# WGLab/DeepMod

Hardware: AMD Instinct MI355X
Metric: base-positions/sec (whole node), E. coli 5mC wd21/f7 BiLSTM (higher is better)
Workload: dtype f16x3

## Files before the change

### deepmod_amd/_lib.py

```python
from __future__ import annotations

import ctypes
import os
from typing import Optional

os.environ.setdefault("HSA_ENABLE_IPC_MODE_LEGACY", "0")

HERE = os.path.dirname(os.path.abspath(__file__))
LIB_PATH = os.path.join(HERE, "csrc", "libdeepmod_hip.so")

DM_OPT_PROFILE = 1
DM_OPT_PRECISION = 2
DM_OPT_ASYNC = 3
DM_OPT_RESERVED_CUS = 4
DM_OPT_F16X3_SHAPE = 5
DM_PREC_F32 = 0
DM_PREC_F16X3 = 1
DM_PREC_F16I8 = 3
DM_PREC_F16X3_ROLES = 2
DM_INFO_PRECISION, DM_INFO_F16_REPRESENTABLE, DM_INFO_F16_LENGTH_SHIFT, DM_INFO_DEVICE, DM_INFO_HAS_F16X3_ROLES = 1, 2, 3, 4, 5
DM_INFO_HAS_F16S = 6
DM_OK, DM_EINVAL, DM_EDEVICE, DM_ENOMEM, DM_ESTATE, DM_ERCCL, DM_ERANGE = 0, -1, -2, -3, -4, -5, -6
(DM_MAP_STATUS, DM_MAP_N_ROWS, DM_MAP_LEFTCLIP, DM_MAP_RIGHTCLIP, DM_MAP_EV_LO, DM_MAP_EV_HI, DM_MAP_FIRST_MATCH_POS,
 DM_MAP_LAST_MATCH_POS, DM_MAP_NUM_INSERT, DM_MAP_NUM_DELETE, DM_MAP_NUM_MISMATCH, DM_MAP_STRAND, DM_MAP_POS_AFTER_CLIP,
 DM_MAP_EVENTS_AFTER_CLIP) = range(14)
DM_MAP_INFO_LEN = 16
DM_MAP_OK, DM_MAP_NO_MATCH, DM_MAP_NEED_ROWS = 0, 1, 2
DM_MOVE_OK, DM_MOVE_COUNT, DM_MOVE_OUTSIDE = 0, 1, 2
(DM_XY_OK, DM_XY_LESS_EVENT, DM_XY_NO_SITE, DM_XY_FILTERED, DM_XY_NO_MATCH, DM_XY_INDEX_ERROR, DM_XY_NEED_ROWS) = range(7)
DM_XY_INFO_LEN = 8
(DM_XY_STATUS, DM_XY_N_ROWS, DM_XY_STRAND, DM_XY_START_CLIP, DM_XY_END_CLIP, DM_XY_POS_AFTER_CLIP, DM_XY_EVENTS_AFTER_CLIP) = range(7)
DM_WEIGHT_FLOATS = 408402

_c = ctypes
_vp = ctypes.c_void_p
_i64 = ctypes.c_int64
# ... 167 lines not shown
```

### deepmod_amd/csrc/deepmod_hip.hip

```cpp
#include "kernels.h"

#include <dlfcn.h>
#include <rccl/rccl.h>

#include <algorithm>
#include <cmath>
#include <cstdarg>
#include <cstdint>
#include <cstdio>
#include <cstring>
#include <string>
#include <utility>
#include <thread>
#include <type_traits>
#include <vector>

#include "../../include/deepmod_hip.h"
#include "head.hip.inc"

using dmk::Packed16;
using dmk::Packed32;

namespace {

// ... 886 lines not shown
}

int dm_model_sync(dm_model* m) {
    if (!m) return fail(DM_EINVAL, "null model");
    HIP_TRY(hipSetDevice(m->device));
    return sync_and_check(m);
}

int dm_model_get_info(dm_model* m, int key, int64_t* value) {
    if (!m || !value) return fail(DM_EINVAL, "null argument");
    switch (key) {
        case DM_INFO_PRECISION: *value = m->precision; return DM_OK;
        case DM_INFO_F16_REPRESENTABLE: *value = m->f16_ok ? 1 : 0; return DM_OK;
        case DM_INFO_F16_LENGTH_SHIFT: *value = m->len_shift; return DM_OK;
        case DM_INFO_DEVICE: *value = m->device; return DM_OK;
        case DM_INFO_HAS_F16S:
#ifdef DM_WITH_F16S
            *value = 1;
#else
            *value = 0;
#endif
            return DM_OK;
        case DM_INFO_HAS_F16X3_ROLES:
#ifdef DM_WITH_F16X3_ROLES
            *value = 1;
#else
            *value = 0;
#endif
            return DM_OK;
        default: return fail(DM_EINVAL, "unknown info key %d", key);
// ... 630 lines not shown
```

### deepmod_amd/csrc/kernels.h

```cpp
#pragma once
#include <hip/hip_runtime.h>

#if defined(DM16Q_ABL_NOCELL) || defined(DM16Q_ABL_NODMA) || defined(DM16Q_ABL_MIX1) || defined(DM16Q_ABL_I8T) || defined(DM16Q_ABL_NOBAR) || defined(DM16Q_ABL_NOVMWAIT) || defined(DM16Q_AINIT) || defined(DM16Q_DEBUG_NOP) ||           \
    defined(DM16Q_NOCHUNK) || defined(DM16Q_NOPN) || defined(DM16Q_LOPACK) || defined(DM16Q_PRE) || defined(DM16Q_SNAKE) || defined(DM16Q_TRANS_COST) ||                     \
    defined(DM16S_ABL_2PROD) || defined(DM16S_ABL_B64) || defined(DM16S_ABL_LO_ONLY) || defined(DM16S_ABL_MFMA16) ||                              \
    defined(DM16S_ABL_MFMA16_PAD) || defined(DM16S_ABL_NOBAR) || defined(DM16S_ABL_NOCELL) || defined(DM16S_ABL_NODMA) ||                          \
    defined(DM16S_ABL_NOLDSA) || defined(DM16S_ADIST) || defined(DM16S_ALO_TRUNC) || defined(DM16S_PRE) || defined(DM_ABL_NOBAR) ||                \
    defined(DM_ABL_NODMA) || defined(DM_ABL_NOEPI) || defined(DM_ABL_NOSEQ) || defined(DM_TIMING) || defined(DM_TRACE) || defined(DM_TRACE2) ||   \
    defined(DM_WLO_TRUNC_ENV) || defined(DM_WLO_TRUNC_DEFAULT) || defined(DM_WITH_F16X3_ROLES) || defined(DM16R_DMA_M) ||                         \
    defined(DM_F16X3_SHAPE_DEFAULT) || defined(DM_WAVES) || defined(DM_MT) || defined(DM_WITH_F16S)
#define DM_ANY_EXPERIMENT_SWITCH 1
#ifndef DM_EXPERIMENT
#error "an ablation / experiment macro is defined without -DDM_EXPERIMENT: timing-only kernels must not be built into the product by a stray -D"
#endif
#else
#define DM_ANY_EXPERIMENT_SWITCH 0
#endif


#if defined(DM_WITH_F16X3_ROLES) && !defined(DM_WITH_F16S)
#error "the roles experiment lives in the translation unit of the 32x32x16 kernels: build it with -DDM_WITH_F16S as well"
#endif

#include <algorithm>
// ... 94 lines not shown
```

### deepmod_amd/csrc/lstm_f16q.hip.inc

```
#ifndef DM16Q_TRANS_COST
#define DM16Q_TRANS_COST 2
#endif
namespace lstm16q {

using lstmc::floatx2;
using lstmc::floatx4;
using lstmc::halfx2;
using lstmc::halfx8;
using lstmc::uintx4;
using lstmc::Params;
using lstmc::ex2;
using lstmc::rcp;
using lstmc::min60;
using lstmc::split_pack;
using lstmc::static_for;
using lstmc::as_h8;

constexpr int HID = 100, NFEAT = 7, WIN = 21, LIVE = 11;
constexpr int NTILE = 13;
constexpr int WAVES = 4, THREADS = 64 * WAVES, TILE_M = 32 * WAVES;
constexpr int KS_L0 = 4, KS_L12 = 7;
constexpr int REC_BYTES = 4096;
constexpr int MIX_BYTES = 2048;
constexpr int TILE_BYTES_L0 = (KS_L0 - 1) * REC_BYTES + 2 * MIX_BYTES, TILE_BYTES_L12 = (KS_L12 - 1) * REC_BYTES + MIX_BYTES;
constexpr int SLOT_BYTES = TILE_BYTES_L12;
constexpr int NSLOT = 2;
constexpr int C2_WAVE_BYTES = NTILE * 1024;
constexpr int C2_LAYER_BYTES = WAVES * C2_WAVE_BYTES;
constexpr size_t LDS_BYTES = size_t(NSLOT) * SLOT_BYTES + C2_LAYER_BYTES;
constexpr size_t LDS_BYTES_I8 = LDS_BYTES + C2_LAYER_BYTES;
constexpr size_t WEIGHT_BYTES_DIR = size_t(NTILE) * (TILE_BYTES_L0 + 2 * TILE_BYTES_L12);
constexpr size_t WEIGHT_BYTES = 2 * WEIGHT_BYTES_DIR;

using lstmc::intx4;
using lstmc::I8_MAGIC;
using lstmc::I8_HI_SCALE;
using lstmc::I8_LO_SCALE;
struct CellPipe {
    float ef[4], ei[4], ej[4], eo[4], t0[4], t1[4];
    unsigned hi01, hi23, lo01, lo23, i01, i23;
    floatx2 fold[2];
    floatx2 kmagic, khi, klo;
    static constexpr int NM = 14;
    template <int PRE, int FMT>
    __device__ static constexpr int nops(int M) {
// ... 142 lines not shown
        return;
#endif
        if constexpr (C < NCH) {
            constexpr int LO = chunk_lo<PRE, FMT>(C, NCH), HI = chunk_lo<PRE, FMT>(C + 1, NCH);
            static_for<HI - LO>([&](auto kc) {
                constexpr int k = LO + decltype(kc)::value;
                this->template op<op_m<PRE, FMT>(k), op_j<PRE, FMT>(k), FMT>(g, gi, S, c2, only_a);
            });
        }
    }
    template <int PRE, int FMT>
    __device__ __forceinline__ void all(floatx4 (&g)[4], const intx4 (&gi)[4], const floatx2 (&S)[2], float* c2, const bool only_a) { chunk<0, 1, PRE, FMT>(g, gi, S, c2, only_a); }
};

template <int TILE_BYTES>
__device__ __forceinline__ void stage_tile(const unsigned char* gtile , unsigned lds_slot , int wave_s, unsigned lane16) {
#ifdef DM16Q_ABL_NODMA
    return;
#endif
    constexpr int NKB = TILE_BYTES / 1024, BASE = NKB / WAVES, REM = NKB % WAVES;
    static_assert(TILE_BYTES % 1024 == 0 && BASE >= 1 && BASE + (REM ? 1 : 0) <= 7, "pieces per wave");
    const int kb0 = wave_s * BASE + (wave_s < REM ? wave_s : REM);
    const unsigned char* g = gtile + kb0 * 1024 + 4096;
    const unsigned l = lds_slot + unsigned(kb0) * 1024u + 4096u;
    unsigned keep;
    asm volatile("s_mov_b32 %0, m0\n\ts_mov_b32 m0, %1\n\ts_nop 0" : "=&s"(keep) : "s"(l) : "memory");
#define DM_PIECE(J) if constexpr ((J) < BASE) asm volatile("global_load_lds_dwordx4 %0, %1 offset:%2" :: "v"(lane16), "s"(g), "i"((J) * 1024 - 4096) : "memory");
    DM_PIECE(0) DM_PIECE(1) DM_PIECE(2) DM_PIECE(3) DM_PIECE(4) DM_PIECE(5) DM_PIECE(6)
#undef DM_PIECE
    if constexpr (REM > 0) {
        asm volatile("s_cmp_lt_i32 %3, %4\n\ts_cbranch_scc0 .Ldm16q_skip_%=\n\tglobal_load_lds_dwordx4 %0, %1 offset:%2\n.Ldm16q_skip_%=:"
                     :: "v"(lane16), "s"(g), "i"(BASE * 1024 - 4096), "s"(wave_s), "i"(REM) : "memory", "scc");
    }
    asm volatile("s_mov_b32 m0, %0" :: "s"(keep) : "memory");
}

struct AQuad {
    halfx8 hiA, loA, hiB, loB;
};
template <int OFF, bool WITH_B, int MIXED>
__device__ __forceinline__ void load_a(AQuad& a, const unsigned addr) {
    if constexpr (MIXED == 0) {
        asm volatile("ds_read_b128 %0, %1 offset:%2" : "=v"(a.hiA) : "v"(addr), "i"(OFF));
        asm volatile("ds_read_b128 %0, %1 offset:%2" : "=v"(a.loA) : "v"(addr), "i"(OFF + 1024));
        if constexpr (WITH_B) {
// ... 11 lines not shown
}
__host__ __device__ constexpr int a_reads(bool with_b, int mixed) { return (mixed == 1 ? 1 : 2) * (with_b ? 2 : 1); }
template <int N>
__device__ __forceinline__ void wait_a(AQuad& a) {
    asm volatile("s_waitcnt lgkmcnt(%4)" : "+v"(a.hiA), "+v"(a.loA), "+v"(a.hiB), "+v"(a.loB) : "i"(N));
}

#define DM16Q_STR2(X) #X
#define DM16Q_STR(X) DM16Q_STR2(X)
#if defined(DM16Q_NOPN)
#define DM16Q_AFTER_MFMA "s_nop " DM16Q_STR(DM16Q_NOPN)
#elif defined(DM16Q_DEBUG_NOP)
#define DM16Q_AFTER_MFMA "s_nop 15\n\ts_nop 15"
#else
#define DM16Q_AFTER_MFMA ""
#endif
#ifndef DM16Q_PRE
#define DM16Q_PRE 2
#endif

template <int LAYER, bool FIRST>
struct StageKind {
    static constexpr bool L0 = LAYER == 0;
    static constexpr int KS_FULL = L0 ? KS_L0 : KS_L12;
    static constexpr int KS = FIRST ? KS_FULL - 3 : KS_FULL;
    static constexpr int TILE_BYTES = L0 ? TILE_BYTES_L0 : TILE_BYTES_L12;
    static constexpr int DMA_OFF = FIRST ? 3 * REC_BYTES : 0;
    static constexpr int DMA_BYTES = TILE_BYTES - DMA_OFF;
    static constexpr int rec_off(int i) { return (FIRST ? 3 + i : i) * REC_BYTES; }
    static constexpr int mixed(int i) { return i == KS - 1 ? (L0 ? 2 : 1) : 0; }
// ... 3 lines not shown

constexpr int quad(int t, int hh, int part) { return (t * 2 + hh) * 2 + part; }

struct WaveState {
    uintx4 own[3][12];
    unsigned m12[3][2][2];
    uintx4 nxt[12];
    float c2reg[NTILE][4];
    float c1reg[NTILE][4];
    floatx4 acc[3][4];
    intx4 acci[3][4];
    floatx2 i8s[3][2];
    CellPipe cp;
    float xf[2][2];
    int slot;
};

template <int LAYER, int MM>
__device__ __forceinline__ void c2_load(WaveState& w, const unsigned c2lds, const int tile, float (&row)[4]) {
    if constexpr (LAYER == 2) {
#pragma unroll
        for (int q = 0; q < 4; ++q) row[q] = w.c2reg[tile][q];
    } else if constexpr (LAYER == 1 && MM == 0) {
#pragma unroll
        for (int q = 0; q < 4; ++q) row[q] = w.c1reg[tile][q];
    } else {
        floatx4 v;
        asm volatile("ds_read_b128 %0, %1 offset:%2" : "=v"(v) : "v"(c2lds), "i"(LAYER * C2_LAYER_BYTES));
#pragma unroll
        for (int q = 0; q < 4; ++q) row[q] = v[q];
    }
// ... 2 lines not shown
__device__ __forceinline__ void c2_store(WaveState& w, const unsigned c2lds, const int tile, const float (&row)[4]) {
    if constexpr (LAYER == 2) {
#pragma unroll
        for (int q = 0; q < 4; ++q) w.c2reg[tile][q] = row[q];
    } else if constexpr (LAYER == 1 && MM == 0) {
#pragma unroll
        for (int q = 0; q < 4; ++q) w.c1reg[tile][q] = row[q];
    } else {
        asm volatile("ds_write_b128 %0, %1 offset:%2" :: "v"(c2lds), "v"(floatx4{row[0], row[1], row[2], row[3]}), "i"(LAYER * C2_LAYER_BYTES) : "memory");
    }
}

__device__ __forceinline__ unsigned lo_lo(unsigned a, unsigned b) { return __builtin_amdgcn_perm(b, a, 0x05040100u); }
__device__ __forceinline__ unsigned hi_lo(unsigned a, unsigned b) { return __builtin_amdgcn_alignbit(b, a, 16); }

template <int LAYER, bool FIRST, int MM>
__device__ __forceinline__ void run_stage(const Params& p, WaveState& w, const unsigned lds_base, const unsigned c2_wave, const unsigned char* wdir, const int dir, const int s,
                                          const float* xwin0, const float* xwin1, const int wave_s, const unsigned lane16, const int grp, const unsigned one2) {
    using K = StageKind<LAYER, FIRST>;
    constexpr bool L0 = K::L0;
    constexpr int KS = K::KS;
    constexpr int PREV = (LAYER + 2) % 3;
    constexpr int I8 = (MM == 1 && !(L0 && FIRST)) ? 1 : 0;
    constexpr int PRE = I8;
    constexpr int PPRE = (MM == 1 && !(PREV == 0 && FIRST)) ? 1 : 0;
    constexpr int FMT = MM == 0 ? 0 : (LAYER == 2 ? 2 : 1);
    constexpr size_t LAYER_OFF[3] = {0, size_t(NTILE) * TILE_BYTES_L0, size_t(NTILE) * (TILE_BYTES_L0 + TILE_BYTES_L12)};
    uintx4 (&own)[12] = w.own[LAYER];
    const uintx4 (&inp)[12] = w.own[L0 ? 0 : LAYER - 1];
    const floatx2 (&S)[2] = w.i8s[LAYER];
    const floatx2 (&PS)[2] = w.i8s[PREV];
    uintx4 mx[2], mx2[2];
    unsigned x0p[2] = {0u, 0u}, x1a[2] = {0u, 0u}, x1b[2] = {0u, 0u};
    if constexpr (L0) {
        bool bad = false;
#pragma unroll
        for (int hh = 0; hh < 2; ++hh) {
// ... 14 lines not shown
        if (bad) *p.range_flag = 1;
        if (s + 1 < LIVE) {
            const int row = dir == 0 ? s + 1 : WIN - 2 - s;
            const int f1 = 4 + grp < NFEAT ? 4 + grp : NFEAT - 1;
            w.xf[0][0] = xwin0[row * NFEAT + grp]; w.xf[0][1] = xwin0[row * NFEAT + f1];
            w.xf[1][0] = xwin1[row * NFEAT + grp]; w.xf[1][1] = xwin1[row * NFEAT + f1];
        }
    }
    const bool last_stage = LAYER == 2 && s == LIVE - 1;
    static_for<NTILE>([&](auto Tc) {
        constexpr int T = decltype(Tc)::value;
        constexpr int P = T == 0 ? NTILE - 1 : T - 1;
        constexpr int accT = T == NTILE - 1 ? 2 : (T & 1), accP = P == NTILE - 1 ? 2 : (P & 1);
        constexpr bool WITH_B = T < NTILE - 1;
        constexpr int NMF = (WITH_B ? 4 : 2) * (I8 ? 2 : 3);
        float c2row[4];
        if constexpr (T == 0) c2_load<PREV, MM>(w, c2_wave + unsigned(NTILE - 1) * 1024u, NTILE - 1, c2row);
        else c2_load<LAYER, MM>(w, c2_wave + unsigned(P) * 1024u, P, c2row);
        const unsigned a_addr = lds_base + unsigned(w.slot) * SLOT_BYTES + lane16;
#ifdef DM16Q_AINIT
        AQuad a[2] = {};
#else
        AQuad a[2];
#endif
        load_a<K::rec_off(0), WITH_B, K::mixed(0)>(a[0], a_addr);
        if (!(last_stage && T == NTILE - 1)) {
            if constexpr (T + 1 < NTILE) {
                unsigned toff = unsigned(T + 1) * K::TILE_BYTES;
                asm volatile("" : "+s"(toff));
                stage_tile<K::DMA_BYTES>(wdir + (LAYER_OFF[LAYER] + K::DMA_OFF) + toff, lds_base + unsigned(w.slot ^ 1) * SLOT_BYTES + K::DMA_OFF, wave_s, lane16);
            } else {
                using KN = StageKind<(LAYER + 1) % 3, FIRST && LAYER < 2>;
                stage_tile<KN::DMA_BYTES>(wdir + (LAYER_OFF[(LAYER + 1) % 3] + KN::DMA_OFF), lds_base + unsigned(w.slot ^ 1) * SLOT_BYTES + KN::DMA_OFF, wave_s, lane16);
            }
        }
        floatx4 (&d)[4] = w.acc[accT];
        intx4 (&di)[4] = w.acci[accT];
        floatx4 (&g)[4] = w.acc[accP];
        const intx4 (&gi)[4] = w.acci[accP];
        const floatx4 z4 = {0.f, 0.f, 0.f, 0.f};
        const intx4 zi4 = {0, 0, 0, 0};
        constexpr int NCH = DM16Q_PRE + NMF * (KS - 1);
#ifdef DM16Q_NOCHUNK
#define DM_CHUNK(C) do { if constexpr ((C) == NCH - 1) { if constexpr (T == 0) w.cp.template all<PPRE, 0>(g, gi, PS, c2row, true); else w.cp.template all<PRE, FMT>(g, gi, S, c2row, false); } } while (0)
#else
#define DM_CHUNK(C) do { if constexpr (T == 0) w.cp.template chunk<(C), NCH, PPRE, 0>(g, gi, PS, c2row, true); else w.cp.template chunk<(C), NCH, PRE, FMT>(g, gi, S, c2row, false); } while (0)
#endif
        if constexpr (KS > 1) static_for<DM16Q_PRE>([&](auto cc) { DM_CHUNK(decltype(cc)::value); });
        static_for<KS>([&](auto ic) {
            constexpr int i = decltype(ic)::value;
            constexpr int MIXED = K::mixed(i);
            if constexpr (i + 1 < KS) load_a<K::rec_off(i + 1), WITH_B, K::mixed(i + 1)>(a[(i + 1) & 1], a_addr);
            if constexpr (i == KS - 1) {
                if constexpr (KS == 1) {
                    if constexpr (T == 0) w.cp.template all<PPRE, 0>(g, gi, PS, c2row, true);
                    else w.cp.template all<PRE, FMT>(g, gi, S, c2row, false);
                }
#ifdef DM16Q_ABL_NOCELL
                w.cp.hi01 = w.cp.hi23 = 0x2E662E66u; w.cp.lo01 = w.cp.lo23 = 0x0A660A66u;
#endif
                if constexpr (T == 0) {
                    w.m12[PREV][0][0] = lo_lo(w.cp.hi01, w.cp.hi01); w.m12[PREV][0][1] = lo_lo(w.cp.hi01, w.cp.lo01);
                    w.m12[PREV][1][0] = lo_lo(w.cp.hi23, w.cp.hi23); w.m12[PREV][1][1] = lo_lo(w.cp.hi23, w.cp.lo23);
                    c2_store<PREV, MM>(w, c2_wave + unsigned(NTILE - 1) * 1024u, NTILE - 1, c2row);
                } else {
                    constexpr int pt = P >> 2, pr = P & 3;
                    unsigned s01, s23;
// ... 14 lines not shown
                    }
                });
            }
            if constexpr (MIXED != 0 && T == 0) {
#pragma unroll
                for (int hh = 0; hh < 2; ++hh) {
                    unsigned in_hl;
                    if constexpr (L0) in_hl = x0p[hh];
                    else in_hl = w.m12[LAYER - 1][hh][1];
                    unsigned own_hh = w.m12[LAYER][hh][0], own_hl = w.m12[LAYER][hh][1];
                    asm volatile("" : "+v"(own_hh), "+v"(own_hl), "+v"(in_hl));
                    mx[hh] = uintx4{own_hh, hi_lo(own_hl, in_hl), in_hl, one2};
                    if constexpr (L0) mx2[hh] = uintx4{x1a[hh], x1b[hh], 0u, 0u};
                }
            }
            wait_a<(i + 1 < KS ? a_reads(WITH_B, K::mixed(i + 1 < KS ? i + 1 : i)) : 0)>(a[i & 1]);
            constexpr int C0 = DM16Q_PRE + NMF * i;
#define DM_MF(AOP, BOP, Q, NO)                                                                                              \
            d[Q] = __builtin_amdgcn_mfma_f32_16x16x32_f16(AOP, BOP, (i == 0 && (NO) == 0) ? z4 : d[Q], 0, 0, 0);              \
            asm volatile(DM16Q_AFTER_MFMA : "+v"(d[Q]) : "v"(AOP), "v"(BOP));
#define DM_MI(AOP, BOP, Q)                                                                                                  \
            di[Q] = __builtin_amdgcn_mfma_i32_16x16x64_i8(__builtin_bit_cast(intx4, AOP), __builtin_bit_cast(intx4, BOP), i == 0 ? zi4 : di[Q], 0, 0, 0); \
            asm volatile(DM16Q_AFTER_MFMA : "+v"(di[Q]) : "v"(AOP), "v"(BOP));
#define DM_CELLQ(N_) if constexpr (KS > 1 && i < KS - 1) DM_CHUNK(C0 + (N_))
            if constexpr (MIXED != 0) {
                const halfx8 b0 = as_h8(mx[0]), b1 = as_h8(mx[1]);
                DM_MF(a[i & 1].hiA, b0, 0, 0)
                DM_MF(a[i & 1].hiA, b1, 2, 0)
                if constexpr (WITH_B) { DM_MF(a[i & 1].hiB, b0, 1, 0) DM_MF(a[i & 1].hiB, b1, 3, 0) }
                if constexpr (MIXED == 2) {
                    const halfx8 e0 = as_h8(mx2[0]), e1 = as_h8(mx2[1]);
                    DM_MF(a[i & 1].loA, e0, 0, 1)
                    DM_MF(a[i & 1].loA, e1, 2, 1)
                    if constexpr (WITH_B) { DM_MF(a[i & 1].loB, e0, 1, 1) DM_MF(a[i & 1].loB, e1, 3, 1) }
                }
            } else {
                constexpr int t = K::opnd(i);
                halfx8 bh[2], bl[2];
#pragma unroll
                for (int hh = 0; hh < 2; ++hh) {
                    if constexpr (K::is_own(i)) { bh[hh] = as_h8(own[quad(t, hh, 0)]); bl[hh] = as_h8(own[quad(t, hh, 1)]); }
                    else { bh[hh] = as_h8(inp[quad(t, hh, 0)]); bl[hh] = as_h8(inp[quad(t, hh, 1)]); }
                }
                if constexpr (I8) {
                    DM_MF(a[i & 1].hiA, bh[0], 0, 0) DM_CELLQ(0);
                    DM_MF(a[i & 1].hiA, bh[1], 2, 0) DM_CELLQ(1);
                    if constexpr (WITH_B) { DM_MF(a[i & 1].hiB, bh[0], 1, 0) DM_CELLQ(2); DM_MF(a[i & 1].hiB, bh[1], 3, 0) DM_CELLQ(3); }
                    DM_MI(a[i & 1].loA, bl[0], 0) DM_CELLQ(WITH_B ? 4 : 2);
                    DM_MI(a[i & 1].loA, bl[1], 2) DM_CELLQ(WITH_B ? 5 : 3);
                    if constexpr (WITH_B) { DM_MI(a[i & 1].loB, bl[0], 1) DM_CELLQ(6); DM_MI(a[i & 1].loB, bl[1], 3) DM_CELLQ(7); }
                } else {
#ifdef DM16Q_SNAKE
                DM_MF(a[i & 1].hiA, bh[0], 0, 0) DM_CELLQ(0);
                if constexpr (WITH_B) { DM_MF(a[i & 1].hiB, bh[0], 1, 0) DM_CELLQ(1); DM_MF(a[i & 1].hiB, bh[1], 3, 0) DM_CELLQ(2); }
                DM_MF(a[i & 1].hiA, bh[1], 2, 0) DM_CELLQ(WITH_B ? 3 : 1);
                DM_MF(a[i & 1].loA, bh[1], 2, 1) DM_CELLQ(WITH_B ? 4 : 2);
                if constexpr (WITH_B) { DM_MF(a[i & 1].loB, bh[1], 3, 1) DM_CELLQ(5); DM_MF(a[i & 1].loB, bh[0], 1, 1) DM_CELLQ(6); }
                DM_MF(a[i & 1].loA, bh[0], 0, 1) DM_CELLQ(WITH_B ? 7 : 3);
                DM_MF(a[i & 1].hiA, bl[0], 0, 2) DM_CELLQ(WITH_B ? 8 : 4);
                if constexpr (WITH_B) { DM_MF(a[i & 1].hiB, bl[0], 1, 2) DM_CELLQ(9); DM_MF(a[i & 1].hiB, bl[1], 3, 2) DM_CELLQ(10); }
                DM_MF(a[i & 1].hiA, bl[1], 2, 2) DM_CELLQ(WITH_B ? 11 : 5);
#else
                DM_MF(a[i & 1].hiA, bh[0], 0, 0) DM_CELLQ(0);
                DM_MF(a[i & 1].hiA, bh[1], 2, 0) DM_CELLQ(1);
                if constexpr (WITH_B) { DM_MF(a[i & 1].hiB, bh[0], 1, 0) DM_CELLQ(2); DM_MF(a[i & 1].hiB, bh[1], 3, 0) DM_CELLQ(3); }
#ifdef DM16Q_ABL_I8T
                DM_MI(a[i & 1].loA, bl[0], 0) DM_CELLQ(WITH_B ? 4 : 2); DM_CELLQ(WITH_B ? 5 : 3);
                DM_MI(a[i & 1].loA, bl[1], 2) DM_CELLQ(WITH_B ? 6 : 4); DM_CELLQ(WITH_B ? 7 : 5);
                if constexpr (WITH_B) { DM_MI(a[i & 1].loB, bl[0], 1) DM_CELLQ(8); DM_CELLQ(9); DM_MI(a[i & 1].loB, bl[1], 3) DM_CELLQ(10); DM_CELLQ(11); }
#else
                DM_MF(a[i & 1].loA, bh[0], 0, 1) DM_CELLQ(WITH_B ? 4 : 2);
                DM_MF(a[i & 1].loA, bh[1], 2, 1) DM_CELLQ(WITH_B ? 5 : 3);
                if constexpr (WITH_B) { DM_MF(a[i & 1].loB, bh[0], 1, 1) DM_CELLQ(6); DM_MF(a[i & 1].loB, bh[1], 3, 1) DM_CELLQ(7); }
                DM_MF(a[i & 1].hiA, bl[0], 0, 2) DM_CELLQ(WITH_B ? 8 : 4);
                DM_MF(a[i & 1].hiA, bl[1], 2, 2) DM_CELLQ(WITH_B ? 9 : 5);
                if constexpr (WITH_B) { DM_MF(a[i & 1].hiB, bl[0], 1, 2) DM_CELLQ(10); DM_MF(a[i & 1].hiB, bl[1], 3, 2) DM_CELLQ(11); }
#endif
#endif
                }
            }
#undef DM_MF
#undef DM_MI
#undef DM_CELLQ
        });
#undef DM_CHUNK
#ifndef DM16Q_ABL_NOVMWAIT
        asm volatile("s_waitcnt vmcnt(0)" ::: "memory");
#endif
#ifndef DM16Q_ABL_NOBAR
        __builtin_amdgcn_s_barrier();
#endif
        w.slot ^= 1;
    });
}

template <int MM>
__global__ __launch_bounds__(THREADS, 1) void bilstm_f16q_kernel(const Params p) {
    extern __shared__ __attribute__((aligned(16))) unsigned char lds16q[];
    const int lane = threadIdx.x & 63;
    const int wave = threadIdx.x >> 6;
    const int wave_s = __builtin_amdgcn_readfirstlane(wave);
    const int grp = lane >> 4, n16 = lane & 15;
    const unsigned lane16 = unsigned(lane) * 16u;
    const unsigned lds_base = (unsigned)(size_t)lds16q;
    const unsigned c2_wave = lds_base + unsigned(NSLOT) * SLOT_BYTES + unsigned(wave) * C2_WAVE_BYTES + lane16;
    const unsigned one2 = grp == 0 ? 0x3C003C00u : 0u;
    const int nwork = 2 * p.ntiles;
    for (int work = blockIdx.x; work < nwork; work += gridDim.x) {
        const int tile = work >> 1, dir = work & 1;
        const long long tile0 = (long long)tile * TILE_M;
        const long long w_out = tile0 + wave * 32 + n16;
        long long wi0 = w_out, wi1 = w_out + 16;
        if (wi0 > p.n - 1) wi0 = p.n - 1;
        if (wi1 > p.n - 1) wi1 = p.n - 1;
        const float* xwin0 = p.x + (p.widx ? (long long)p.widx[wi0] : wi0) * p.xstride;
        const float* xwin1 = p.x + (p.widx ? (long long)p.widx[wi1] : wi1) * p.xstride;
        const unsigned char* wdir = p.wpack + size_t(dir) * WEIGHT_BYTES_DIR;

        WaveState w;
#pragma unroll
// ... 36 lines not shown
            for (int t = 0; t < NTILE; ++t) {
                asm volatile("ds_write_b128 %0, %1" :: "v"(c2_wave + unsigned(t * 1024)), "v"(z4) : "memory");
                if constexpr (MM == 1) asm volatile("ds_write_b128 %0, %1 offset:%2" :: "v"(c2_wave + unsigned(t * 1024)), "v"(z4), "i"(C2_LAYER_BYTES) : "memory");
            }
        }
        {
            using K0 = StageKind<0, true>;
            stage_tile<K0::DMA_BYTES>(wdir + K0::DMA_OFF, lds_base + K0::DMA_OFF, wave_s, lane16);
        }
        {
            const int row = dir == 0 ? 0 : WIN - 1;
            const int f1 = 4 + grp < NFEAT ? 4 + grp : NFEAT - 1;
            w.xf[0][0] = xwin0[row * NFEAT + grp]; w.xf[0][1] = xwin0[row * NFEAT + f1];
            w.xf[1][0] = xwin1[row * NFEAT + grp]; w.xf[1][1] = xwin1[row * NFEAT + f1];
        }
        asm volatile("s_waitcnt vmcnt(0) lgkmcnt(0)" ::: "memory");
        __syncthreads();

#define DM_STAGE(LAYER, FIRST, S_) run_stage<LAYER, FIRST, MM>(p, w, lds_base, c2_wave, wdir, dir, S_, xwin0, xwin1, wave_s, lane16, grp, one2)
        DM_STAGE(0, true, 0);
        DM_STAGE(1, true, 0);
        DM_STAGE(2, true, 0);
        for (int s = 1; s < LIVE; ++s) {
            DM_STAGE(0, false, s);
            DM_STAGE(1, false, s);
            DM_STAGE(2, false, s);
        }
#undef DM_STAGE
        {
            float c2row[4];
#pragma unroll
            for (int q = 0; q < 4; ++q) c2row[q] = w.c2reg[NTILE - 1][q];
            w.cp.template all<MM, 0>(w.acc[2], w.acci[2], w.i8s[2], c2row, true);
            w.m12[2][0][1] = lo_lo(w.cp.hi01, w.cp.lo01);
            w.m12[2][1][1] = lo_lo(w.cp.hi23, w.cp.lo23);
#pragma unroll
            for (int q = 0; q < 12; ++q) w.own[2][q] = w.nxt[q];
        }
#pragma unroll
        for (int hh = 0; hh < 2; ++hh) {
            float hsum0 = 0.0f, hsum1 = 0.0f;
            static_for<NTILE>([&](auto Sc) {
                constexpr int S = decltype(Sc)::value;
// ... 27 lines not shown
```

### include/deepmod_hip.h

```cpp
#ifndef DEEPMOD_HIP_H
#define DEEPMOD_HIP_H

#include <stddef.h>
#include <stdint.h>

#ifdef __cplusplus
extern "C" {
#endif

#define DM_OK 0
#define DM_EINVAL (-1)
#define DM_EDEVICE (-2)
#define DM_ENOMEM (-3)
#define DM_ESTATE (-4)
#define DM_ERCCL (-5)
#define DM_ERANGE (-6)

#define DM_NFEAT 7
#define DM_HIDDEN 100
#define DM_WINDOW 21
#define DM_LAYERS 3
#define DM_WEIGHT_FLOATS 408402

#define DM_OPT_PROFILE 1
#define DM_OPT_PRECISION 2
#define DM_OPT_ASYNC 3
#define DM_OPT_RESERVED_CUS 4
#define DM_OPT_F16X3_SHAPE 5
#define DM_PREC_F32 0
#define DM_PREC_F16X3 1
#define DM_PREC_F16X3_ROLES 2
#define DM_PREC_F16I8 3
#define DM_INFO_PRECISION 1
#define DM_INFO_F16_REPRESENTABLE 2
#define DM_INFO_F16_LENGTH_SHIFT 3
#define DM_INFO_DEVICE 4
#define DM_INFO_HAS_F16X3_ROLES 5
#define DM_INFO_HAS_F16S 6

typedef struct dm_model dm_model;
typedef struct dm_summary dm_summary;

const char* dm_last_error(void);
const char* dm_version(void);

const char* dm_build_flags(void);

int dm_device_count(void);
int dm_device_pci_bus_id(int device, char* buf, int len);

dm_model* dm_model_create(int device, const float* weights, size_t n_floats, int n_feat, int hidden,
                          int window, int layers);
void dm_model_destroy(dm_model* m);
// ... 234 lines not shown
```

Before: 47.81 million.

## Use a three-slot LDS weight ring with two-tile-ahead DMA in f16x3 kernel

For the f16x3 (MM==0) path, the weight staging buffer in LDS grows from two slots to three. Weight tiles are prefetched two tiles ahead, and the wait at the end of each tile becomes a partial vmcnt wait plus a barrier. The next tile's A fragments and c2 row are loaded before the current tile's MFMAs finish, so the per-tile full drain is removed and LDS reads overlap with compute. In exchange it uses more LDS (which may cut occupancy), holds more registers for the carried A fragments, and adds a compile-time parity bookkeeping. It also adds optional experimental piece-splitting of the DMA and a grid-cap info query.

```diff
diff --git a/deepmod_amd/_lib.py b/deepmod_amd/_lib.py
--- a/deepmod_amd/_lib.py
+++ b/deepmod_amd/_lib.py
@@ -20,6 +20,7 @@
 DM_PREC_F16X3_ROLES = 2
 DM_INFO_PRECISION, DM_INFO_F16_REPRESENTABLE, DM_INFO_F16_LENGTH_SHIFT, DM_INFO_DEVICE, DM_INFO_HAS_F16X3_ROLES = 1, 2, 3, 4, 5
 DM_INFO_HAS_F16S = 6
+DM_INFO_GRID_CAP = 7
 DM_OK, DM_EINVAL, DM_EDEVICE, DM_ENOMEM, DM_ESTATE, DM_ERCCL, DM_ERANGE = 0, -1, -2, -3, -4, -5, -6
 (DM_MAP_STATUS, DM_MAP_N_ROWS, DM_MAP_LEFTCLIP, DM_MAP_RIGHTCLIP, DM_MAP_EV_LO, DM_MAP_EV_HI, DM_MAP_FIRST_MATCH_POS,
  DM_MAP_LAST_MATCH_POS, DM_MAP_NUM_INSERT, DM_MAP_NUM_DELETE, DM_MAP_NUM_MISMATCH, DM_MAP_STRAND, DM_MAP_POS_AFTER_CLIP,
diff --git a/deepmod_amd/csrc/deepmod_hip.hip b/deepmod_amd/csrc/deepmod_hip.hip
--- a/deepmod_amd/csrc/deepmod_hip.hip
+++ b/deepmod_amd/csrc/deepmod_hip.hip
@@ -924,6 +924,7 @@
         case DM_INFO_F16_REPRESENTABLE: *value = m->f16_ok ? 1 : 0; return DM_OK;
         case DM_INFO_F16_LENGTH_SHIFT: *value = m->len_shift; return DM_OK;
         case DM_INFO_DEVICE: *value = m->device; return DM_OK;
+        case DM_INFO_GRID_CAP: *value = m->grid_cap; return DM_OK;
         case DM_INFO_HAS_F16S:
 #ifdef DM_WITH_F16S
             *value = 1;
diff --git a/deepmod_amd/csrc/kernels.h b/deepmod_amd/csrc/kernels.h
--- a/deepmod_amd/csrc/kernels.h
+++ b/deepmod_amd/csrc/kernels.h
@@ -2,7 +2,7 @@
 #include <hip/hip_runtime.h>
 
 #if defined(DM16Q_ABL_NOCELL) || defined(DM16Q_ABL_NODMA) || defined(DM16Q_ABL_MIX1) || defined(DM16Q_ABL_I8T) || defined(DM16Q_ABL_NOBAR) || defined(DM16Q_ABL_NOVMWAIT) || defined(DM16Q_AINIT) || defined(DM16Q_DEBUG_NOP) ||           \
-    defined(DM16Q_NOCHUNK) || defined(DM16Q_NOPN) || defined(DM16Q_LOPACK) || defined(DM16Q_PRE) || defined(DM16Q_SNAKE) || defined(DM16Q_TRANS_COST) ||                     \
+    defined(DM16Q_NOCHUNK) || defined(DM16Q_PIECES) || defined(DM16Q_NOPN) || defined(DM16Q_LOPACK) || defined(DM16Q_PRE) || defined(DM16Q_SNAKE) || defined(DM16Q_TRANS_COST) ||                     \
     defined(DM16S_ABL_2PROD) || defined(DM16S_ABL_B64) || defined(DM16S_ABL_LO_ONLY) || defined(DM16S_ABL_MFMA16) ||                              \
     defined(DM16S_ABL_MFMA16_PAD) || defined(DM16S_ABL_NOBAR) || defined(DM16S_ABL_NOCELL) || defined(DM16S_ABL_NODMA) ||                          \
     defined(DM16S_ABL_NOLDSA) || defined(DM16S_ADIST) || defined(DM16S_ALO_TRUNC) || defined(DM16S_PRE) || defined(DM_ABL_NOBAR) ||                \
diff --git a/deepmod_amd/csrc/lstm_f16q.hip.inc b/deepmod_amd/csrc/lstm_f16q.hip.inc
--- a/deepmod_amd/csrc/lstm_f16q.hip.inc
+++ b/deepmod_amd/csrc/lstm_f16q.hip.inc
@@ -24,11 +24,13 @@
 constexpr int MIX_BYTES = 2048;
 constexpr int TILE_BYTES_L0 = (KS_L0 - 1) * REC_BYTES + 2 * MIX_BYTES, TILE_BYTES_L12 = (KS_L12 - 1) * REC_BYTES + MIX_BYTES;
 constexpr int SLOT_BYTES = TILE_BYTES_L12;
-constexpr int NSLOT = 2;
+template <int MM>
+constexpr int NSLOT = MM == 0 ? 3 : 2;
 constexpr int C2_WAVE_BYTES = NTILE * 1024;
 constexpr int C2_LAYER_BYTES = WAVES * C2_WAVE_BYTES;
-constexpr size_t LDS_BYTES = size_t(NSLOT) * SLOT_BYTES + C2_LAYER_BYTES;
-constexpr size_t LDS_BYTES_I8 = LDS_BYTES + C2_LAYER_BYTES;
+constexpr size_t LDS_BYTES = size_t(NSLOT<0>) * SLOT_BYTES + C2_LAYER_BYTES;
+constexpr size_t LDS_BYTES_I8 = size_t(NSLOT<1>) * SLOT_BYTES + 2 * C2_LAYER_BYTES;
+static_assert(LDS_BYTES <= 163840 && LDS_BYTES_I8 <= 163840, "LDS of one CU");
 constexpr size_t WEIGHT_BYTES_DIR = size_t(NTILE) * (TILE_BYTES_L0 + 2 * TILE_BYTES_L12);
 constexpr size_t WEIGHT_BYTES = 2 * WEIGHT_BYTES_DIR;
 
@@ -201,21 +203,25 @@
 };
 
 template <int TILE_BYTES>
+constexpr int PIECES_BASE = TILE_BYTES / 1024 / WAVES;
+template <int TILE_BYTES, int PART = 0, int NPART = 1>
 __device__ __forceinline__ void stage_tile(const unsigned char* gtile , unsigned lds_slot , int wave_s, unsigned lane16) {
 #ifdef DM16Q_ABL_NODMA
     return;
 #endif
     constexpr int NKB = TILE_BYTES / 1024, BASE = NKB / WAVES, REM = NKB % WAVES;
+    constexpr int LO = BASE * PART / NPART, HI = BASE * (PART + 1) / NPART;
+    if constexpr (LO == HI && !(REM > 0 && PART == NPART - 1)) return;
     static_assert(TILE_BYTES % 1024 == 0 && BASE >= 1 && BASE + (REM ? 1 : 0) <= 7, "pieces per wave");
     const int kb0 = wave_s * BASE + (wave_s < REM ? wave_s : REM);
     const unsigned char* g = gtile + kb0 * 1024 + 4096;
     const unsigned l = lds_slot + unsigned(kb0) * 1024u + 4096u;
     unsigned keep;
     asm volatile("s_mov_b32 %0, m0\n\ts_mov_b32 m0, %1\n\ts_nop 0" : "=&s"(keep) : "s"(l) : "memory");
-#define DM_PIECE(J) if constexpr ((J) < BASE) asm volatile("global_load_lds_dwordx4 %0, %1 offset:%2" :: "v"(lane16), "s"(g), "i"((J) * 1024 - 4096) : "memory");
+#define DM_PIECE(J) if constexpr ((J) >= LO && (J) < HI) asm volatile("global_load_lds_dwordx4 %0, %1 offset:%2" :: "v"(lane16), "s"(g), "i"((J) * 1024 - 4096) : "memory");
     DM_PIECE(0) DM_PIECE(1) DM_PIECE(2) DM_PIECE(3) DM_PIECE(4) DM_PIECE(5) DM_PIECE(6)
 #undef DM_PIECE
-    if constexpr (REM > 0) {
+    if constexpr (REM > 0 && PART == NPART - 1) {
         asm volatile("s_cmp_lt_i32 %3, %4\n\ts_cbranch_scc0 .Ldm16q_skip_%=\n\tglobal_load_lds_dwordx4 %0, %1 offset:%2\n.Ldm16q_skip_%=:"
                      :: "v"(lane16), "s"(g), "i"(BASE * 1024 - 4096), "s"(wave_s), "i"(REM) : "memory", "scc");
     }
@@ -257,6 +263,9 @@
 #define DM16Q_AFTER_MFMA "s_nop 15\n\ts_nop 15"
 #else
 #define DM16Q_AFTER_MFMA ""
+#endif
+#ifndef DM16Q_PIECES
+#define DM16Q_PIECES 0
 #endif
 #ifndef DM16Q_PRE
 #define DM16Q_PRE 2
@@ -290,7 +299,11 @@
     CellPipe cp;
     float xf[2][2];
     int slot;
+    AQuad a[2];
+    floatx4 c2n;
 };
+
+__host__ __device__ constexpr bool c2_in_lds(int layer, int mm) { return !(layer == 2 || (layer == 1 && mm == 0)); }
 
 template <int LAYER, int MM>
 __device__ __forceinline__ void c2_load(WaveState& w, const unsigned c2lds, const int tile, float (&row)[4]) {
@@ -323,13 +336,14 @@
 __device__ __forceinline__ unsigned lo_lo(unsigned a, unsigned b) { return __builtin_amdgcn_perm(b, a, 0x05040100u); }
 __device__ __forceinline__ unsigned hi_lo(unsigned a, unsigned b) { return __builtin_amdgcn_alignbit(b, a, 16); }
 
-template <int LAYER, bool FIRST, int MM>
+template <int LAYER, bool FIRST, int MM, int E>
 __device__ __forceinline__ void run_stage(const Params& p, WaveState& w, const unsigned lds_base, const unsigned c2_wave, const unsigned char* wdir, const int dir, const int s,
                                           const float* xwin0, const float* xwin1, const int wave_s, const unsigned lane16, const int grp, const unsigned one2) {
     using K = StageKind<LAYER, FIRST>;
     constexpr bool L0 = K::L0;
     constexpr int KS = K::KS;
     constexpr int PREV = (LAYER + 2) % 3;
+    constexpr bool RING3 = NSLOT<MM> == 3;
     constexpr int I8 = (MM == 1 && !(L0 && FIRST)) ? 1 : 0;
     constexpr int PRE = I8;
     constexpr int PPRE = (MM == 1 && !(PREV == 0 && FIRST)) ? 1 : 0;
@@ -374,25 +388,48 @@
         constexpr int accT = T == NTILE - 1 ? 2 : (T & 1), accP = P == NTILE - 1 ? 2 : (P & 1);
         constexpr bool WITH_B = T < NTILE - 1;
         constexpr int NMF = (WITH_B ? 4 : 2) * (I8 ? 2 : 3);
+        using KN = StageKind<(LAYER + 1) % 3, FIRST && LAYER < 2>;
+        constexpr int EP = RING3 ? (E + T * KS) & 1 : 0;
         float c2row[4];
-        if constexpr (T == 0) c2_load<PREV, MM>(w, c2_wave + unsigned(NTILE - 1) * 1024u, NTILE - 1, c2row);
+        if constexpr (RING3 && c2_in_lds(T == 0 ? PREV : LAYER, MM)) {
+#pragma unroll
+            for (int q = 0; q < 4; ++q) c2row[q] = w.c2n[q];
+        } else if constexpr (T == 0) c2_load<PREV, MM>(w, c2_wave + unsigned(NTILE - 1) * 1024u, NTILE - 1, c2row);
         else c2_load<LAYER, MM>(w, c2_wave + unsigned(P) * 1024u, P, c2row);
         const unsigned a_addr = lds_base + unsigned(w.slot) * SLOT_BYTES + lane16;
 #ifdef DM16Q_AINIT
-        AQuad a[2] = {};
+        AQuad a_tile[2] = {};
 #else
-        AQuad a[2];
-#endif
-        load_a<K::rec_off(0), WITH_B, K::mixed(0)>(a[0], a_addr);
-        if (!(last_stage && T == NTILE - 1)) {
-            if constexpr (T + 1 < NTILE) {
-                unsigned toff = unsigned(T + 1) * K::TILE_BYTES;
-                asm volatile("" : "+s"(toff));
-                stage_tile<K::DMA_BYTES>(wdir + (LAYER_OFF[LAYER] + K::DMA_OFF) + toff, lds_base + unsigned(w.slot ^ 1) * SLOT_BYTES + K::DMA_OFF, wave_s, lane16);
-            } else {
-                using KN = StageKind<(LAYER + 1) % 3, FIRST && LAYER < 2>;
-                stage_tile<KN::DMA_BYTES>(wdir + (LAYER_OFF[(LAYER + 1) % 3] + KN::DMA_OFF), lds_base + unsigned(w.slot ^ 1) * SLOT_BYTES + KN::DMA_OFF, wave_s, lane16);
-            }
+        AQuad a_tile[2];
+#endif
+        AQuad (&a)[2] = RING3 ? w.a : a_tile;
+        const int slot_next = w.slot == 2 ? 0 : w.slot + 1;
+        auto dma_ahead = [&](auto PARTc, auto NPARTc) {
+            constexpr int PART = decltype(PARTc)::value, NPART = decltype(NPARTc)::value;
+            if (!(last_stage && T >= NTILE - 2)) {
+                const unsigned dst = lds_base + unsigned(w.slot == 0 ? 2 : w.slot - 1) * SLOT_BYTES;
+                if constexpr (T + 2 < NTILE) {
+                    unsigned toff = unsigned(T + 2) * K::TILE_BYTES;
+                    asm volatile("" : "+s"(toff));
+                    stage_tile<K::DMA_BYTES, PART, NPART>(wdir + (LAYER_OFF[LAYER] + K::DMA_OFF) + toff, dst + K::DMA_OFF, wave_s, lane16);
+                } else {
+                    stage_tile<KN::DMA_BYTES, PART, NPART>(wdir + (LAYER_OFF[(LAYER + 1) % 3] + KN::DMA_OFF + size_t(T + 2 - NTILE) * KN::TILE_BYTES), dst + KN::DMA_OFF, wave_s, lane16);
+                }
+            }
+        };
+        if constexpr (!RING3) {
+            load_a<K::rec_off(0), WITH_B, K::mixed(0)>(a[0], a_addr);
+            if (!(last_stage && T == NTILE - 1)) {
+                if constexpr (T + 1 < NTILE) {
+                    unsigned toff = unsigned(T + 1) * K::TILE_BYTES;
+                    asm volatile("" : "+s"(toff));
+                    stage_tile<K::DMA_BYTES>(wdir + (LAYER_OFF[LAYER] + K::DMA_OFF) + toff, lds_base + unsigned(w.slot ^ 1) * SLOT_BYTES + K::DMA_OFF, wave_s, lane16);
+                } else {
+                    stage_tile<KN::DMA_BYTES>(wdir + (LAYER_OFF[(LAYER + 1) % 3] + KN::DMA_OFF), lds_base + unsigned(w.slot ^ 1) * SLOT_BYTES + KN::DMA_OFF, wave_s, lane16);
+                }
+            }
+        } else {
+            if constexpr (DM16Q_PIECES == 0 || KS == 1) dma_ahead(std::integral_constant<int, 0>{}, std::integral_constant<int, 1>{});
         }
         floatx4 (&d)[4] = w.acc[accT];
         intx4 (&di)[4] = w.acci[accT];
@@ -410,7 +447,8 @@
         static_for<KS>([&](auto ic) {
             constexpr int i = decltype(ic)::value;
             constexpr int MIXED = K::mixed(i);
-            if constexpr (i + 1 < KS) load_a<K::rec_off(i + 1), WITH_B, K::mixed(i + 1)>(a[(i + 1) & 1], a_addr);
+            constexpr int ab = (i + EP) & 1;
+            if constexpr (i + 1 < KS) load_a<K::rec_off(i + 1), WITH_B, K::mixed(i + 1)>(a[ab ^ 1], a_addr);
             if constexpr (i == KS - 1) {
                 if constexpr (KS == 1) {
                     if constexpr (T == 0) w.cp.template all<PPRE, 0>(g, gi, PS, c2row, true);
@@ -455,7 +493,21 @@
                     if constexpr (L0) mx2[hh] = uintx4{x1a[hh], x1b[hh], 0u, 0u};
                 }
             }
-            wait_a<(i + 1 < KS ? a_reads(WITH_B, K::mixed(i + 1 < KS ? i + 1 : i)) : 0)>(a[i & 1]);
+            wait_a<(i + 1 < KS ? a_reads(WITH_B, K::mixed(i + 1 < KS ? i + 1 : i)) : 0)>(a[ab]);
+            if constexpr (RING3 && i == KS - 1) {
+                constexpr int VMB = (LAYER == 2 && T >= NTILE - 2) ? 0 : (T + 2 < NTILE ? PIECES_BASE<K::DMA_BYTES> : PIECES_BASE<KN::DMA_BYTES>);
+#ifndef DM16Q_ABL_NOVMWAIT
+                asm volatile("s_waitcnt vmcnt(%0)" :: "i"(VMB) : "memory");
+#endif
+#ifndef DM16Q_ABL_NOBAR
+                asm volatile("s_barrier" ::: "memory");
+#endif
+                if constexpr (c2_in_lds(LAYER, MM)) asm volatile("ds_read_b128 %0, %1 offset:%2" : "=v"(w.c2n) : "v"(c2_wave + unsigned(T) * 1024u), "i"(LAYER * C2_LAYER_BYTES));
+                const unsigned n_addr = lds_base + unsigned(slot_next) * SLOT_BYTES + lane16;
+                constexpr bool NEXT_B = T + 1 != NTILE - 1;
+                if constexpr (T + 1 < NTILE) load_a<K::rec_off(0), NEXT_B, K::mixed(0)>(a[ab ^ 1], n_addr);
+                else load_a<KN::rec_off(0), NEXT_B, KN::mixed(0)>(a[ab ^ 1], n_addr);
+            }
             constexpr int C0 = DM16Q_PRE + NMF * i;
 #define DM_MF(AOP, BOP, Q, NO)                                                                                              \
             d[Q] = __builtin_amdgcn_mfma_f32_16x16x32_f16(AOP, BOP, (i == 0 && (NO) == 0) ? z4 : d[Q], 0, 0, 0);              \
@@ -463,17 +515,20 @@
 #define DM_MI(AOP, BOP, Q)                                                                                                  \
             di[Q] = __builtin_amdgcn_mfma_i32_16x16x64_i8(__builtin_bit_cast(intx4, AOP), __builtin_bit_cast(intx4, BOP), i == 0 ? zi4 : di[Q], 0, 0, 0); \
             asm volatile(DM16Q_AFTER_MFMA : "+v"(di[Q]) : "v"(AOP), "v"(BOP));
-#define DM_CELLQ(N_) if constexpr (KS > 1 && i < KS - 1) DM_CHUNK(C0 + (N_))
+#define DM_CELLQ(N_) do { if constexpr (KS > 1 && i < KS - 1) DM_CHUNK(C0 + (N_)); DM_PIECE_AT(N_); } while (0)
+#define DM_PIECE_AT(N_) do { if constexpr (RING3 && DM16Q_PIECES == 3 && KS > 1 && i < 2 && (WITH_B ? (N_) % 3 == 1 : ((N_) >= 1 && (N_) <= 4))) {      \
+                constexpr int pp = 4 * i + (WITH_B ? ((N_) - 1) / 3 : (N_) - 1);                                                                      \
+                if constexpr (pp < 7) dma_ahead(std::integral_constant<int, pp>{}, std::integral_constant<int, 7>{}); } } while (0)
             if constexpr (MIXED != 0) {
                 const halfx8 b0 = as_h8(mx[0]), b1 = as_h8(mx[1]);
-                DM_MF(a[i & 1].hiA, b0, 0, 0)
-                DM_MF(a[i & 1].hiA, b1, 2, 0)
-                if constexpr (WITH_B) { DM_MF(a[i & 1].hiB, b0, 1, 0) DM_MF(a[i & 1].hiB, b1, 3, 0) }
+                DM_MF(a[ab].hiA, b0, 0, 0)
+                DM_MF(a[ab].hiA, b1, 2, 0)
+                if constexpr (WITH_B) { DM_MF(a[ab].hiB, b0, 1, 0) DM_MF(a[ab].hiB, b1, 3, 0) }
                 if constexpr (MIXED == 2) {
                     const halfx8 e0 = as_h8(mx2[0]), e1 = as_h8(mx2[1]);
-                    DM_MF(a[i & 1].loA, e0, 0, 1)
-                    DM_MF(a[i & 1].loA, e1, 2, 1)
-                    if constexpr (WITH_B) { DM_MF(a[i & 1].loB, e0, 1, 1) DM_MF(a[i & 1].loB, e1, 3, 1) }
+                    DM_MF(a[ab].loA, e0, 0, 1)
+                    DM_MF(a[ab].loA, e1, 2, 1)
+                    if constexpr (WITH_B) { DM_MF(a[ab].loB, e0, 1, 1) DM_MF(a[ab].loB, e1, 3, 1) }
                 }
             } else {
                 constexpr int t = K::opnd(i);
@@ -484,38 +539,39 @@
                     else { bh[hh] = as_h8(inp[quad(t, hh, 0)]); bl[hh] = as_h8(inp[quad(t, hh, 1)]); }
                 }
                 if constexpr (I8) {
-                    DM_MF(a[i & 1].hiA, bh[0], 0, 0) DM_CELLQ(0);
-                    DM_MF(a[i & 1].hiA, bh[1], 2, 0) DM_CELLQ(1);
-                    if constexpr (WITH_B) { DM_MF(a[i & 1].hiB, bh[0], 1, 0) DM_CELLQ(2); DM_MF(a[i & 1].hiB, bh[1], 3, 0) DM_CELLQ(3); }
-                    DM_MI(a[i & 1].loA, bl[0], 0) DM_CELLQ(WITH_B ? 4 : 2);
-                    DM_MI(a[i & 1].loA, bl[1], 2) DM_CELLQ(WITH_B ? 5 : 3);
-                    if constexpr (WITH_B) { DM_MI(a[i & 1].loB, bl[0], 1) DM_CELLQ(6); DM_MI(a[i & 1].loB, bl[1], 3) DM_CELLQ(7); }
+                    DM_MF(a[ab].hiA, bh[0], 0, 0) DM_CELLQ(0);
+                    DM_MF(a[ab].hiA, bh[1], 2, 0) DM_CELLQ(1);
+                    if constexpr (WITH_B) { DM_MF(a[ab].hiB, bh[0], 1, 0) DM_CELLQ(2); DM_MF(a[ab].hiB, bh[1], 3, 0) DM_CELLQ(3); }
+                    DM_MI(a[ab].loA, bl[0], 0) DM_CELLQ(WITH_B ? 4 : 2);
+                    DM_MI(a[ab].loA, bl[1], 2) DM_CELLQ(WITH_B ? 5 : 3);
+                    if constexpr (WITH_B) { DM_MI(a[ab].loB, bl[0], 1) DM_CELLQ(6); DM_MI(a[ab].loB, bl[1], 3) DM_CELLQ(7); }
                 } else {
 #ifdef DM16Q_SNAKE
-                DM_MF(a[i & 1].hiA, bh[0], 0, 0) DM_CELLQ(0);
-                if constexpr (WITH_B) { DM_MF(a[i & 1].hiB, bh[0], 1, 0) DM_CELLQ(1); DM_MF(a[i & 1].hiB, bh[1], 3, 0) DM_CELLQ(2); }
-                DM_MF(a[i & 1].hiA, bh[1], 2, 0) DM_CELLQ(WITH_B ? 3 : 1);
-                DM_MF(a[i & 1].loA, bh[1], 2, 1) DM_CELLQ(WITH_B ? 4 : 2);
-                if constexpr (WITH_B) { DM_MF(a[i & 1].loB, bh[1], 3, 1) DM_CELLQ(5); DM_MF(a[i & 1].loB, bh[0], 1, 1) DM_CELLQ(6); }
-                DM_MF(a[i & 1].loA, bh[0], 0, 1) DM_CELLQ(WITH_B ? 7 : 3);
-                DM_MF(a[i & 1].hiA, bl[0], 0, 2) DM_CELLQ(WITH_B ? 8 : 4);
-                if constexpr (WITH_B) { DM_MF(a[i & 1].hiB, bl[0], 1, 2) DM_CELLQ(9); DM_MF(a[i & 1].hiB, bl[1], 3, 2) DM_CELLQ(10); }
-                DM_MF(a[i & 1].hiA, bl[1], 2, 2) DM_CELLQ(WITH_B ? 11 : 5);
+                DM_MF(a[ab].hiA, bh[0], 0, 0) DM_CELLQ(0);
+                if constexpr (WITH_B) { DM_MF(a[ab].hiB, bh[0], 1, 0) DM_CELLQ(1); DM_MF(a[ab].hiB, bh[1], 3, 0) DM_CELLQ(2); }
+                DM_MF(a[ab].hiA, bh[1], 2, 0) DM_CELLQ(WITH_B ? 3 : 1);
+                DM_MF(a[ab].loA, bh[1], 2, 1) DM_CELLQ(WITH_B ? 4 : 2);
+                if constexpr (WITH_B) { DM_MF(a[ab].loB, bh[1], 3, 1) DM_CELLQ(5); DM_MF(a[ab].loB, bh[0], 1, 1) DM_CELLQ(6); }
+                DM_MF(a[ab].loA, bh[0], 0, 1) DM_CELLQ(WITH_B ? 7 : 3);
+                DM_MF(a[ab].hiA, bl[0], 0, 2) DM_CELLQ(WITH_B ? 8 : 4);
+                if constexpr (WITH_B) { DM_MF(a[ab].hiB, bl[0], 1, 2) DM_CELLQ(9); DM_MF(a[ab].hiB, bl[1], 3, 2) DM_CELLQ(10); }
+                DM_MF(a[ab].hiA, bl[1], 2, 2) DM_CELLQ(WITH_B ? 11 : 5);
 #else
-                DM_MF(a[i & 1].hiA, bh[0], 0, 0) DM_CELLQ(0);
-                DM_MF(a[i & 1].hiA, bh[1], 2, 0) DM_CELLQ(1);
-                if constexpr (WITH_B) { DM_MF(a[i & 1].hiB, bh[0], 1, 0) DM_CELLQ(2); DM_MF(a[i & 1].hiB, bh[1], 3, 0) DM_CELLQ(3); }
+                DM_MF(a[ab].hiA, bh[0], 0, 0) DM_CELLQ(0);
+                DM_MF(a[ab].hiA, bh[1], 2, 0) DM_CELLQ(1);
+                if constexpr (WITH_B) { DM_MF(a[ab].hiB, bh[0], 1, 0) DM_CELLQ(2); DM_MF(a[ab].hiB, bh[1], 3, 0) DM_CELLQ(3); }
 #ifdef DM16Q_ABL_I8T
-                DM_MI(a[i & 1].loA, bl[0], 0) DM_CELLQ(WITH_B ? 4 : 2); DM_CELLQ(WITH_B ? 5 : 3);
-                DM_MI(a[i & 1].loA, bl[1], 2) DM_CELLQ(WITH_B ? 6 : 4); DM_CELLQ(WITH_B ? 7 : 5);
-                if constexpr (WITH_B) { DM_MI(a[i & 1].loB, bl[0], 1) DM_CELLQ(8); DM_CELLQ(9); DM_MI(a[i & 1].loB, bl[1], 3) DM_CELLQ(10); DM_CELLQ(11); }
+                DM_MI(a[ab].loA, bl[0], 0) DM_CELLQ(WITH_B ? 4 : 2); DM_CELLQ(WITH_B ? 5 : 3);
+                DM_MI(a[ab].loA, bl[1], 2) DM_CELLQ(WITH_B ? 6 : 4); DM_CELLQ(WITH_B ? 7 : 5);
+                if constexpr (WITH_B) { DM_MI(a[ab].loB, bl[0], 1) DM_CELLQ(8); DM_CELLQ(9); DM_MI(a[ab].loB, bl[1], 3) DM_CELLQ(10); DM_CELLQ(11); }
 #else
-                DM_MF(a[i & 1].loA, bh[0], 0, 1) DM_CELLQ(WITH_B ? 4 : 2);
-                DM_MF(a[i & 1].loA, bh[1], 2, 1) DM_CELLQ(WITH_B ? 5 : 3);
-                if constexpr (WITH_B) { DM_MF(a[i & 1].loB, bh[0], 1, 1) DM_CELLQ(6); DM_MF(a[i & 1].loB, bh[1], 3, 1) DM_CELLQ(7); }
-                DM_MF(a[i & 1].hiA, bl[0], 0, 2) DM_CELLQ(WITH_B ? 8 : 4);
-                DM_MF(a[i & 1].hiA, bl[1], 2, 2) DM_CELLQ(WITH_B ? 9 : 5);
-                if constexpr (WITH_B) { DM_MF(a[i & 1].hiB, bl[0], 1, 2) DM_CELLQ(10); DM_MF(a[i & 1].hiB, bl[1], 3, 2) DM_CELLQ(11); }
+                DM_MF(a[ab].loA, bh[0], 0, 1) DM_CELLQ(WITH_B ? 4 : 2);
+                DM_MF(a[ab].loA, bh[1], 2, 1) DM_CELLQ(WITH_B ? 5 : 3);
+                if constexpr (WITH_B) { DM_MF(a[ab].loB, bh[0], 1, 1) DM_CELLQ(6); DM_MF(a[ab].loB, bh[1], 3, 1) DM_CELLQ(7); }
+                if constexpr (RING3 && DM16Q_PIECES == 2 && KS > 1 && i < 2) dma_ahead(std::integral_constant<int, i>{}, std::integral_constant<int, 2>{});
+                DM_MF(a[ab].hiA, bl[0], 0, 2) DM_CELLQ(WITH_B ? 8 : 4);
+                DM_MF(a[ab].hiA, bl[1], 2, 2) DM_CELLQ(WITH_B ? 9 : 5);
+                if constexpr (WITH_B) { DM_MF(a[ab].hiB, bl[0], 1, 2) DM_CELLQ(10); DM_MF(a[ab].hiB, bl[1], 3, 2) DM_CELLQ(11); }
 #endif
 #endif
                 }
@@ -523,15 +579,21 @@
 #undef DM_MF
 #undef DM_MI
 #undef DM_CELLQ
+#undef DM_PIECE_AT
+            if constexpr (RING3 && DM16Q_PIECES == 1 && KS > 1 && i == 0) dma_ahead(std::integral_constant<int, 0>{}, std::integral_constant<int, 1>{});
         });
 #undef DM_CHUNK
+        if constexpr (RING3) {
+            w.slot = slot_next;
+        } else {
 #ifndef DM16Q_ABL_NOVMWAIT
-        asm volatile("s_waitcnt vmcnt(0)" ::: "memory");
+            asm volatile("s_waitcnt vmcnt(0)" ::: "memory");
 #endif
 #ifndef DM16Q_ABL_NOBAR
-        __builtin_amdgcn_s_barrier();
-#endif
-        w.slot ^= 1;
+            __builtin_amdgcn_s_barrier();
+#endif
+            w.slot ^= 1;
+        }
     });
 }
 
@@ -544,7 +606,13 @@
     const int grp = lane >> 4, n16 = lane & 15;
     const unsigned lane16 = unsigned(lane) * 16u;
     const unsigned lds_base = (unsigned)(size_t)lds16q;
-    const unsigned c2_wave = lds_base + unsigned(NSLOT) * SLOT_BYTES + unsigned(wave) * C2_WAVE_BYTES + lane16;
+    constexpr bool RING3 = NSLOT<MM> == 3;
+    using KA0 = StageKind<0, true>; using KA1 = StageKind<1, true>; using KA2 = StageKind<2, true>;
+    using KB0 = StageKind<0, false>; using KB1 = StageKind<1, false>; using KB2 = StageKind<2, false>;
+    constexpr int EA0 = 0, EA1 = (EA0 + NTILE * KA0::KS) & 1, EA2 = (EA1 + NTILE * KA1::KS) & 1;
+    constexpr int EB0 = (EA2 + NTILE * KA2::KS) & 1, EB1 = (EB0 + NTILE * KB0::KS) & 1, EB2 = (EB1 + NTILE * KB1::KS) & 1, EEND = (EB2 + NTILE * KB2::KS) & 1;
+    static_assert(EEND == EB0, "the step loop must hand the A fragments over in the buffer it received them in");
+    const unsigned c2_wave = lds_base + unsigned(NSLOT<MM>) * SLOT_BYTES + unsigned(wave) * C2_WAVE_BYTES + lane16;
     const unsigned one2 = grp == 0 ? 0x3C003C00u : 0u;
     const int nwork = 2 * p.ntiles;
     for (int work = blockIdx.x; work < nwork; work += gridDim.x) {
@@ -611,19 +679,29 @@
             w.xf[0][0] = xwin0[row * NFEAT + grp]; w.xf[0][1] = xwin0[row * NFEAT + f1];
             w.xf[1][0] = xwin1[row * NFEAT + grp]; w.xf[1][1] = xwin1[row * NFEAT + f1];
         }
-        asm volatile("s_waitcnt vmcnt(0) lgkmcnt(0)" ::: "memory");
-        __syncthreads();
-
-#define DM_STAGE(LAYER, FIRST, S_) run_stage<LAYER, FIRST, MM>(p, w, lds_base, c2_wave, wdir, dir, S_, xwin0, xwin1, wave_s, lane16, grp, one2)
-        DM_STAGE(0, true, 0);
-        DM_STAGE(1, true, 0);
-        DM_STAGE(2, true, 0);
+        if constexpr (RING3) {
+            using K0 = StageKind<0, true>;
+            stage_tile<K0::DMA_BYTES>(wdir + K0::DMA_OFF + K0::TILE_BYTES, lds_base + SLOT_BYTES + K0::DMA_OFF, wave_s, lane16);
+            static_assert(K0::DMA_BYTES % (1024 * WAVES) == 0, "every wave issues PIECES_BASE pieces of super-tile 1");
+            asm volatile("s_waitcnt vmcnt(%0) lgkmcnt(0)" :: "i"(PIECES_BASE<K0::DMA_BYTES>) : "memory");
+            asm volatile("s_barrier" ::: "memory");
+            load_a<K0::rec_off(0), true, K0::mixed(0)>(w.a[EA0], lds_base + lane16);
+        } else {
+            asm volatile("s_waitcnt vmcnt(0) lgkmcnt(0)" ::: "memory");
+            __syncthreads();
+        }
+
+#define DM_STAGE(LAYER, FIRST, S_, E_) run_stage<LAYER, FIRST, MM, RING3 ? (E_) : 0>(p, w, lds_base, c2_wave, wdir, dir, S_, xwin0, xwin1, wave_s, lane16, grp, one2)
+        DM_STAGE(0, true, 0, EA0);
+        DM_STAGE(1, true, 0, EA1);
+        DM_STAGE(2, true, 0, EA2);
         for (int s = 1; s < LIVE; ++s) {
-            DM_STAGE(0, false, s);
-            DM_STAGE(1, false, s);
-            DM_STAGE(2, false, s);
+            DM_STAGE(0, false, s, EB0);
+            DM_STAGE(1, false, s, EB1);
+            DM_STAGE(2, false, s, EB2);
         }
 #undef DM_STAGE
+        if constexpr (RING3) wait_a<0>(w.a[EEND]);
         {
             float c2row[4];
 #pragma unroll
diff --git a/include/deepmod_hip.h b/include/deepmod_hip.h
--- a/include/deepmod_hip.h
+++ b/include/deepmod_hip.h
@@ -37,6 +37,7 @@
 #define DM_INFO_DEVICE 4
 #define DM_INFO_HAS_F16X3_ROLES 5
 #define DM_INFO_HAS_F16S 6
+#define DM_INFO_GRID_CAP 7
 
 typedef struct dm_model dm_model;
 typedef struct dm_summary dm_summary;
```

Result: no change. 48.14 million, median of 6 (+0.7%).
